# Hex-Lee/gluon-e2e-asr

Hardware: NVIDIA B200
Metric: ctc_fwd_bwd_valid_frames_per_sec (higher is better)
Workload: dtype f64

## Files before the change

gluon_e2e_asr_b200/csrc/ctcb.cu:

```cuda
#include <cuda_runtime.h>
#include <dlfcn.h>
#include <stdarg.h>
#include <stdio.h>
#include <stdlib.h>
#include <string.h>

#include <mutex>
#include <new>
#include <utility>
#include <vector>

#include "ctcb.h"
#include "ctcb_dlpack.h"
#include "ctcb_kernels.cuh"
#include "ctcb_meet.cuh"
#include "ctcb_grad2.cuh"
#include "ctcb_proj.cuh"

struct ctcb_mailbox {
    int device = 0, rank = 0, world = 0;
    double* local = nullptr;
    void* opened[ctcb::kMailMaxRanks] = {};
    ctcb::MailboxDev dev{};
    ctcb::MailboxDev* dev_d = nullptr;
// ... 14 lines not shown
    cudaLaunchAttribute attr[1];
    attr[0].id = cudaLaunchAttributeProgrammaticStreamSerialization;
    attr[0].val.programmaticStreamSerializationAllowed = 1;
    cfg.attrs = attr; cfg.numAttrs = programmatic ? 1 : 0;
    const ctcb::MailboxDev* md = g_xchg.mb->dev_d;
    cudaLaunchKernelEx(&cfg, ctcb::k_mailbox_exchange, md, g_xchg.values, g_xchg.count, g_xchg.out, 0);
    g_xchg = PendingXchg{};
    return true;
}
thread_local const ctcb_proj_t* g_proj = nullptr;
struct DecodeRequest { int32_t* tokens; int32_t* lengths; int unk; };
thread_local const DecodeRequest* g_decode = nullptr;
thread_local bool g_recompute = false;
thread_local cudaEvent_t* g_prof_events = nullptr;
thread_local int g_prof_count = 0;

enum Opt { OPT_WALK_P, OPT_WALK_NW, OPT_WALK_STAGES, OPT_OVERLAP, OPT_FUSED, OPT_WALK_PER_SM, OPT_EMIT_STAGED,
           OPT_GRAD_STAGED, OPT_MEET, OPT_GRAD2, OPT_GRAD2_BLOCKS, OPT_WALK_HW_WAIT, OPT_GRAD2_OCC, OPT_PROJ_CTAS, OPT_PROJ_DBG, OPT_PROJ_OVERLAP, OPT_MEET_FWD, OPT_WALK_PDL, OPT_GRAD_POLL_NS, OPT_COUNT };
const char* const kOptNames[OPT_COUNT] = {"walk_p", "walk_nw", "walk_stages", "overlap", "fused", "walk_per_sm",
                                          "emit_staged", "grad_staged", "meet", "grad2", "grad2_blocks", "walk_hw_wait", "grad2_occ", "proj_ctas", "proj_dbg", "proj_overlap", "meet_fwd", "walk_pdl", "grad_poll_ns"};
struct Options {
    int v[OPT_COUNT];
    Options() {
        for (int i = 0; i < OPT_COUNT; ++i) {
            char name[64] = "CTCB_";
            size_t k = 5;
            for (const char* c = kOptNames[i]; *c && k + 1 < sizeof(name); ++c) name[k++] = (char)(*c >= 'a' && *c <= 'z' ? *c - 32 : *c);
            name[k] = 0;
            const char* e = getenv(name);
            v[i] = e ? atoi(e) : -1;
// ... 226 lines not shown
}

bool is_device_ptr(const void* ptr) {
    if (!ptr) return true;
    cudaPointerAttributes at{};
    if (cudaPointerGetAttributes(&at, ptr) != cudaSuccess) { cudaGetLastError(); return false; }
    return at.type == cudaMemoryTypeDevice || at.type == cudaMemoryTypeManaged;
}
void* pinned_device_alias(const void* ptr) {
    if (!ptr) return nullptr;
    cudaPointerAttributes at{};
    if (cudaPointerGetAttributes(&at, ptr) != cudaSuccess) { cudaGetLastError(); return nullptr; }
    return at.type == cudaMemoryTypeHost ? at.devicePointer : nullptr;
}

}

extern "C" {

int ctcb_version(void) { return CTCB_VERSION; }
const char* ctcb_last_error(void) { return g_err; }
int ctcb_last_launch_count(void) { return g_launches; }
int ctcb_last_walk_config(int32_t* p, int32_t* nw) {
    if (p) *p = g_walk_p;
    if (nw) *nw = g_walk_nw;
    return CTCB_OK;
}

int ctcb_last_grad_kernel(void) { return g_grad_kernel; }

int ctcb_set_option(const char* name, int32_t value) {
    if (!name) return fail(CTCB_INVALID_VALUE, "option name is NULL");
    for (int i = 0; i < OPT_COUNT; ++i)
// ... 183 lines not shown
        if (lay.off_hA + need <= lay.total) {
            if (p->status) CUDA_TRY(cudaMemsetAsync(p->status, 0, sizeof(int32_t) * (size_t)p->B, stream));
            ctcb::MeetArgs ma{dp, w.hA, lay.NB};
            using MeetFn = void (*)(ctcb::MeetArgs);
            const MeetFn mfn = mp == 1 ? ctcb::k_meet<1> : mp == 2 ? ctcb::k_meet<2> : ctcb::k_meet<4>;
            const size_t msm = ctcb::meet_smem_layout(mp, p->V, lay.Lp).total;
            CUDA_TRY(ensure_dynamic_smem(reinterpret_cast<const void*>(mfn), msm));
            g_walk_p = mp; g_walk_nw = 1; g_grad_kernel = 3;
            mfn<<<p->B, 256, msm, stream>>>(ma);
            mark(stream);
            if (launch_pending_xchg(stream)) mark(stream);
            CUDA_TRY(cudaGetLastError());
            return CTCB_OK;
        }
    }
    if (phases & PH_FORWARD) {
        if (p->status) CUDA_TRY(cudaMemsetAsync(p->status, 0, sizeof(int32_t) * (size_t)p->B, stream));
        const WalkEntry* we = lay.walk;
        if (!we) return fail(CTCB_UNSUPPORTED, "no walker configuration for Lmax=%d", p->Lmax);
        g_walk_p = we->P; g_walk_nw = we->NW;
        int stages = 0;
        if (!pick_stages(lay.W, we->NW, lay.fused ? lay.Lp : 0, &stages))
            return fail(CTCB_UNSUPPORTED, "Lmax=%d V=%d: the emission ring does not fit in shared memory", p->Lmax, p->V);
        const WalkFn wfn = (bf && lay.fused) ? we->fused_bf16[need_grad ? 1 : 0] : we->fn[lay.fused][need_grad ? 1 : 0];
        size_t smem = ctcb::walk_smem_bytes(lay.W, we->NW, stages, lay.fused ? lay.Lp : 0);
        if (lay.fused && need_grad && (phases & PH_BACKWARD) && overlap_allowed(p->B, true)) {
            int dev = 0, nsm = 148;
            cudaGetDevice(&dev);
            cudaDeviceGetAttribute(&nsm, cudaDevAttrMultiProcessorCount, dev);
            int per_sm = (2 * p->B + nsm - 1) / nsm;
// ... 36 lines not shown
                }
#undef EMIT_NQ
#undef EMIT_LAUNCH
            }
            mark(stream);
            return CTCB_OK;
        };
        const bool xchg = !(phases & PH_BACKWARD) && launch_pending_xchg(stream);
        if (xchg) mark(stream);
        const bool beside = g_proj && !need_grad && !xchg && !g_prof_events && opt(OPT_PROJ_OVERLAP) != 0;
        const bool meet_fwd = !need_grad && (opt(OPT_MEET_FWD) >= 0 ? opt(OPT_MEET_FWD) != 0 : (p->B <= 148 && !beside));
        if (meet_fwd) CUDA_TRY(cudaMemsetAsync(w.meetcnt, 0, sizeof(int) * (size_t)p->B, stream));
        auto launch_walk = [&](bool after_xchg, bool beside_proj) -> int {
            ctcb::WalkArgs wa{dp, w, p->T, stages, p->blank, p->loss, p->loss_sum, nullptr, 0, 1, 0, 0, 0};
            wa.beside_proj = beside_proj ? 1 : 0;
            const bool pdl = lay.fused && !after_xchg && !beside_proj && opt(OPT_WALK_PDL) != 0;
            wa.pdl_wait = pdl ? 1 : 0;
            wa.meet = meet_fwd ? 1 : 0;
            wa.hw_wait = opt(OPT_WALK_HW_WAIT) >= 0 ? opt(OPT_WALK_HW_WAIT) : (2 * p->B > 148 ? 1 : 0);
            wa.publish = ((phases & PH_BACKWARD) && !g_prof_events && overlap_allowed(p->B, lay.fused != 0)) ? 1 : 2;
            const int wthreads = (we->NW + (lay.fused ? ctcb::kFusedProducers + 1 : 1)) * 32;
            cudaLaunchConfig_t cfg{};
            cfg.gridDim = dim3(p->B, (need_grad || meet_fwd) ? 2 : 1); cfg.blockDim = dim3(wthreads); cfg.dynamicSmemBytes = smem; cfg.stream = stream;
            cudaLaunchAttribute attr[1];
            attr[0].id = cudaLaunchAttributeProgrammaticStreamSerialization;
            attr[0].val.programmaticStreamSerializationAllowed = 1;
            cfg.attrs = attr; cfg.numAttrs = (after_xchg || pdl) ? 1 : 0;
            CUDA_TRY(cudaLaunchKernelEx(&cfg, wfn, wa));
            mark(stream);
            return CTCB_OK;
// ... 4 lines not shown
        if (int rc = launch_walk((xchg && lay.fused != 0) || beside, beside)) return rc;
        if (g_recompute) {
            CUDA_TRY(ctcb::launch_proj_occ(dp, w, stream));
            mark(stream);
        }
        if (g_decode) {
            const size_t dsm = 2 * sizeof(int) * (size_t)p->T;
            if (dsm > 48 * 1024) CUDA_TRY(ensure_dynamic_smem(reinterpret_cast<const void*>(ctcb::k_greedy_collapse), dsm));
            ctcb::k_greedy_collapse<<<p->B, 256, dsm, stream>>>(w.tflag, w.ntile, p->data_lengths, p->data_lengths_dtype, p->T, p->blank,
                                                                g_decode->unk, g_decode->tokens, g_decode->lengths);
            mark(stream);
        }
    }
    if (phases & PH_BACKWARD) {
        ctcb::GradArgs ga{dp, w};
        const int gpairs = p->Lmax + 1;
        const int gch = gpairs <= 32 ? 1 : gpairs <= 64 ? 2 : gpairs <= 128 ? 4 : gpairs <= 256 ? 8 : gpairs <= 512 ? 16 : 0;
        size_t gsm = ctcb::grad_smem_bytes(lay.Lp, 32 * gch);
        int gthreads = 128;
        if (gsm > 200 * 1024) return fail(CTCB_UNSUPPORTED, "Lmax=%d too long for the gradient kernel", p->Lmax);
        int vec = pick_vec(p->logits, p->logits_stride_t, p->logits_row_offsets ? 0 : p->logits_stride_b, p->V, esz);
        const int gvec = pick_vec(p->grad, p->grad_stride_t, p->grad_stride_b, p->V, esz);
        if (gvec < vec) vec = gvec;
        const int ch = gch;
        const int units = (p->V / vec + 31) / 32;
        const int xq = units <= 1 ? 1 : units <= 2 ? 2 : units <= 4 ? 4 : 0;
        const dim3 ggrid(p->B, lay.NB);
        using GradFn = void (*)(ctcb::GradArgs);
        GradFn gfn = nullptr;
#define GRAD_X(V_, C_, T_) (xq == 1 ? ctcb::k_grad<V_, C_, 1, 0, T_> : xq == 2 ? ctcb::k_grad<V_, C_, 2, 0, T_> : \
// ... 876 lines not shown
```

gluon_e2e_asr_b200/csrc/ctcb_kernels.cuh:

```cuda
#pragma once
#include <cuda_bf16.h>
#include <cuda_runtime.h>
#include <stdint.h>

namespace ctcb {

constexpr int kG = 8;
constexpr int kEC = 10;
constexpr int kD = 100;
constexpr int kDrift = 200;
constexpr int kZeroE = -(1 << 28);
constexpr float kLog2e = 1.4426950408889634f;
constexpr double kLn2 = 0.6931471805599453094;
constexpr float kMinLog2 = -100.0f;
constexpr int kMaxStages = 16;

enum : int { UTT_INFEASIBLE = 1, UTT_BAD_LABEL = 2, UTT_LEN_CLAMPED = 4, UTT_WIDE_LOGITS = 8 };
constexpr long long kSpinLimit = 4000000000LL;
enum : int { DT_I32 = 0, DT_I64 = 1, DT_F32 = 2, DT_F64 = 3 };

struct Problem {
    int T, B, V, Lmax, blank, label_pad;
    const float* logits; long long st_t, st_b;
    const long long* row_off;
// ... 496 lines not shown
    long long* trace;
    int hw_wait;
    int publish;
    int meet;
    int pdl_wait;
    int beside_proj;
};

#ifdef CTCB_TRACE
#define CTCB_TP(id) do { if (a.trace && blockIdx.x == 0 && lane == 0) \
    a.trace[((size_t)(blockIdx.y * 32 + warp) * 4096 + (size_t)n * 8 + (id))] = clock64(); } while (0)
#else
#define CTCB_TP(id) do { } while (0)
#endif

struct HaloMeta { double lm; int el; int R; int F; int pad; };
constexpr int kHaloDepth = 16;

constexpr int kFusedProducers = 2;

__host__ __device__ inline size_t walk_smem_bytes(int W, int NW, int stages, int fused_Lp = 0) {
    return (size_t)stages * kEC * W * sizeof(double) + 2 * kMaxStages * sizeof(uint64_t) +
           (size_t)NW * kHaloDepth * kG * sizeof(double) + (size_t)NW * kHaloDepth * sizeof(HaloMeta) +
           (size_t)NW * sizeof(int) + 64 + (fused_Lp ? 16 + kFusedProducers * 64 + (size_t)fused_Lp * sizeof(int) : 0);
}

template <int P, int NW, int DIR, bool HIST, bool FUSED, typename LT = float>
__device__ __forceinline__ void walk_dir(const WalkArgs& a, unsigned char* smem_raw, int Tb, int Lb, int uflags) {
    constexpr int PW = 32 * P;
    constexpr unsigned FULL = 0xffffffffu;
    const Workspace& w = a.w;
    const int b = blockIdx.x;
    const int tid = threadIdx.x, lane = tid & 31, warp = tid >> 5;
    const int W = w.W, NS = a.stages;
    const int NQ = (Tb + kG - 1) / kG;
    const int rlast = Tb - (NQ - 1) * kG;
    const bool meet = !HIST && a.meet && NQ >= 2;
    const int Mblk = (NQ + 1) / 2;
    const int NQr = meet ? (DIR ? NQ - Mblk : Mblk) : NQ;
    if (!HIST && DIR == 1 && !meet) return;
    const uint32_t stage_bytes = (uint32_t)W * kEC * 8u;

    const uint32_t ring = smem_u32(smem_raw);
// ... 4 lines not shown
    const uint32_t prog = meta + NW * kHaloDepth * (uint32_t)sizeof(HaloMeta);
    const uint32_t lsum = (prog + NW * 4 + 7u) & ~7u;
    int* slab = reinterpret_cast<int*>(smem_raw + (lsum - ring) + 32 + kFusedProducers * 64);

    if (tid == 0) {
        for (int s = 0; s < NS; ++s) { mbar_init(&full[s], 1); mbar_init(&empty[s], NW); }
        asm volatile("fence.mbarrier_init.release.cluster;" ::: "memory");
        sts_s32(lsum + 8, 0);
        if (FUSED) for (int q = 0; q < kFusedProducers * 8; ++q) sts_f64(lsum + 16 + q * 8, 0.0);
    }
    if (tid < NW) sts_s32(prog + tid * 4, 0);
    __syncthreads();

    if (FUSED && warp >= NW && warp < NW + kFusedProducers) {
        const Problem& p = a.p;
        constexpr int CPL = 16;
        const int q = warp - NW, V = p.V;
        const int fj = lane >> 2, qk = lane & 3;
        const int cpl = (V + 3) >> 2, col0 = qk * cpl;
        const LT* base = utt_logits<LT>(p, b);
        const float kMinProb = 7.888609052210118e-31f;
        auto load_blk = [&](int n, float (&x)[CPL]) {
            const int t = (DIR ? NQ - 1 - n : n) * kG + fj;
            const LT* row = base + (long long)t * p.st_t + col0;
            const bool valid = t < Tb;
#pragma unroll
            for (int i = 0; i < CPL; ++i) x[i] = (valid && i < cpl && col0 + i < V) ? ldx(row + i) : -INFINITY;
        };
        float cur[CPL], nxt[CPL];
        double ls = 0.0;
        bool floored = false;
        int n = q;
        if (n < NQr) load_blk(n, cur);
#pragma unroll 1
        for (; n < NQr; n += kFusedProducers) {
            if (n + kFusedProducers < NQr) load_blk(n + kFusedProducers, nxt);
            const int t = (DIR ? NQ - 1 - n : n) * kG + fj;
            const bool valid = t < Tb;
            float mx = cur[0];
#pragma unroll
            for (int i = 1; i < CPL; ++i) mx = fmaxf(mx, cur[i]);
            mx = fmaxf(mx, __shfl_xor_sync(FULL, mx, 1));
            mx = fmaxf(mx, __shfl_xor_sync(FULL, mx, 2));
            float e[CPL], sm = 0.0f;
#pragma unroll
            for (int i = 0; i < CPL; ++i) {
                e[i] = valid ? fast_ex2((cur[i] - mx) * kLog2e) : 0.0f;
                sm += e[i];
// ... 43 lines not shown
            if (c1 > 0) dl[__popc(m0) + __popc(m1 & below)] = make_int2(lane + 32, r1);
            w.runv[(size_t)b * 64 + lane] = make_int2(r0, r0 + c0);
            w.runv[(size_t)b * 64 + lane + 32] = make_int2(r1, r1 + c1);
            for (int j = 0; j < Lb; ++j) {
                const int v = slab[j];
                if (v == lane) rank[j] = r0++;
                else if (v == lane + 32) rank[j] = r1++;
            }
            if (lane == 0) {
                dl[nd] = make_int2(-1, Lb);
                w.nd[b] = nd; w.Tb[b] = Tb; w.Lb[b] = Lb; w.flags[b] = uflags;
            }
            __syncwarp();
            if (lane == 0) st_release_gpu(w.gprog + 4 * b + 2, w.stamp);
        }
        if (HIST && lane == 0 && a.publish) {
            int* gp = w.gprog + 4 * b + DIR;
            const uint32_t last_prog = prog + (NW - 1) * 4;
            int seen = 0;
            while (seen < NQ) {
                const int v = lds_acquire(last_prog);
                if (v > seen) { st_release_gpu(gp, v); seen = v; }
                else __nanosleep(a.publish == 2 ? 4000 : 128);
            }
        }
        (void)p;
        return;
    }

    if (!FUSED && warp == NW) {
        const double* Eb = w.E + (size_t)b * w.NB * W * kEC;
        int tile_seen = -1;
        auto issue = [&](int n, int st) {
            const int blk = DIR ? NQ - 1 - n : n;
            if (a.beside_proj && (blk >> 4) != tile_seen) {
                const int* f = w.tflag + (size_t)b * w.ntile + (blk >> 4);
                const long long t0 = clock64();
                while (ld_acquire_gpu(f) == 0 && clock64() - t0 < kSpinLimit) __nanosleep(256);
// ... 75 lines not shown
    const uint32_t nb_meta = meta + (warp > 0 ? warp - 1 : 0) * kHaloDepth * (uint32_t)sizeof(HaloMeta);
    const uint32_t nb_prog = prog + (warp > 0 ? warp - 1 : 0) * 4;
    double pm = 0.0;
    int c_el = 0, c_R = 0, c_F = 0;
    int Rout = 0, Fout = 0;

    int st = 0, ph = 0;
    uint32_t stage_base = ring;
#pragma unroll 1
    for (int n = 0; n < NQr; ++n) {
        const int blk = DIR ? NQ - 1 - n : n;
        const int ns = blk == NQ - 1 ? rlast : kG;
        const uint32_t par = (uint32_t)(n & (kHaloDepth - 1));
        CTCB_TP(0);
        mbar_wait(&full[st], ph);
        const int j0 = DIR ? ns - 1 : 0;
        double yb, yl[P];
        yb = lds_f64(stage_base + bcol + (uint32_t)j0 * 8u);
#pragma unroll
        for (int p = 0; p < P; ++p) yl[p] = lds_f64(stage_base + ccol[p] + (uint32_t)j0 * 8u);
        int bad = 0;
        {
            constexpr unsigned LO = (1023u - kDrift) << 20, SPAN = (2u * kDrift + 1u) << 20;
#pragma unroll
            for (int p = 0; p < P; ++p) {
                const unsigned hb = (unsigned)__double2hiint(bm[p]), hl = (unsigned)__double2hiint(lm[p]);
                bad |= (int)(hb != 0u) & (int)(hb - LO >= SPAN);
                bad |= (int)(hl != 0u) & (int)(hl - LO >= SPAN);
            }
        }
// ... 150 lines not shown
                step(j, nj, DIR ? 0u - (uint32_t)j * 8u : (uint32_t)j * 8u);
            }
        } else {
#pragma unroll 1
            for (int jj = 0; jj < ns; ++jj) {
                const int j = DIR ? ns - 1 - jj : jj;
                const int nj = jj + 1 < ns ? (DIR ? j - 1 : j + 1) : -1;
                step(j, nj, DIR ? 0u - (uint32_t)j * 8u : (uint32_t)j * 8u);
            }
        }
        CTCB_TP(4);
        __syncwarp();
        if (lane == 31) {
            if (NW > 1 || (FUSED && HIST)) sts_release(prog + warp * 4, n + 1);
            mbar_arrive(&empty[st]);
        }
        CTCB_TP(5);
        CTCB_TP(6);
        stage_base += stage_bytes;
        if (++st == NS) { st = 0; ph ^= 1; stage_base = ring; }
        if (HIST) { hch += DIR ? -kHistStep : kHistStep; och += DIR ? -kOffStep : kOffStep; }
    }

    if (meet) {
        MeetSlot* mine = w.meet + ((size_t)b * 2 + DIR) * (NW * PW) + g0;
#pragma unroll
        for (int p = 0; p < P; ++p) {
            double vb = bm[p], vl = lm[p];
            if (DIR) {
                const double prev = p == 0 ? pm : lm[p - 1];
                const double t0 = fma(bm[p], flb[p], lm[p]);
                vb = fma(prev, fb[p], bm[p]);
                vl = fma(prev, fls[p], t0);
            }
            MeetSlot ms;
            ms.ob = vb != 0.0 ? eb[p] + dexp(vb) : kZeroE; ms.vb = vb != 0.0 ? dmant(vb) : 0.0;
            ms.ol = vl != 0.0 ? el[p] + dexp(vl) : kZeroE; ms.vl = vl != 0.0 ? dmant(vl) : 0.0;
            mine[p] = ms;
// ... 64 lines not shown
                    lz = lds_f64(lsum);
                }
                const double nll = -kLn2 * ((double)eb[p] + log2(sb) - lz);
                a.loss[b] = (float)nll;
                if (a.loss_sum) atomicAdd(a.loss_sum, nll);
            }
        }
    }
}

template <int P, int NW, bool HIST, bool FUSED, typename LT = float>
__global__ void __launch_bounds__((NW + (FUSED ? kFusedProducers + 1 : 1)) * 32) k_walk(WalkArgs a) {
    extern __shared__ __align__(128) unsigned char smem_raw[];
    if (a.pdl_wait) asm volatile("griddepcontrol.wait;" ::: "memory");
    const int b = blockIdx.x;
    if (!FUSED) {
        asm volatile("griddepcontrol.launch_dependents;" ::: "memory");
        if (a.beside_proj) {
            if (threadIdx.x == 0) {
                const long long t0 = clock64();
                while (ld_acquire_gpu(a.w.gprog + 4 * b + 2) != a.w.stamp && clock64() - t0 < kSpinLimit) __nanosleep(256);
            }
            __syncthreads();
        }
        const int flags = __ldcg(a.w.flags + b), Tb = __ldcg(a.w.Tb + b), Lb = __ldcg(a.w.Lb + b);
        if (flags & UTT_INFEASIBLE) return;
        if (blockIdx.y == 0) walk_dir<P, NW, 0, HIST, false>(a, smem_raw, Tb, Lb, flags);
        else                 walk_dir<P, NW, 1, HIST, false>(a, smem_raw, Tb, Lb, flags);
        return;
    }
    const Problem& p = a.p;
    const Workspace& w = a.w;
    const int tid = threadIdx.x, nthr = blockDim.x;
    __shared__ int s_L, s_rep, s_flags;
    if (tid == 0) {
        w.gprog[4 * b + blockIdx.y] = 0;
        if (blockIdx.y == 0) { w.gprog[4 * b + 2] = 0; w.gprog[4 * b + 3] = 0; }
        __threadfence();
        s_L = p.Lmax; s_rep = 0; s_flags = 0;
    }
    __syncthreads();
    asm volatile("griddepcontrol.launch_dependents;" ::: "memory");
    int Tb = p.T, lenflags = 0;
    if (p.data_len) {
        long long t64 = load_as_int(p.data_len, p.data_len_dtype, b);
        if (t64 < 0) { t64 = 0; lenflags = UTT_LEN_CLAMPED; }
        if (t64 > p.T) { t64 = p.T; lenflags = UTT_LEN_CLAMPED; }
        Tb = (int)t64;
    }
    int L;
    if (p.label_len) {
        long long l64 = load_as_int(p.label_len, p.label_len_dtype, b);
        if (l64 < 0) { l64 = 0; lenflags = UTT_LEN_CLAMPED; }
        if (l64 > p.Lmax) { l64 = p.Lmax; lenflags = UTT_LEN_CLAMPED; }
        L = (int)l64;
    } else {
        for (int j = tid; j < p.Lmax; j += nthr)
            if (load_as_int(p.labels, p.label_dtype, b * p.lst_b + j * p.lst_l) == p.label_pad) atomicMin(&s_L, j);
        __syncthreads();
        L = s_L;
    }
    int* slab;
    {
        const size_t stage_bytes = (size_t)w.W * kEC * 8;
        size_t off = (size_t)a.stages * stage_bytes + 2 * kMaxStages * sizeof(uint64_t) +
                     (size_t)NW * kHaloDepth * kG * 8 + (size_t)NW * kHaloDepth * sizeof(HaloMeta) + (size_t)NW * 4;
        off = (off + 7) & ~(size_t)7;
        slab = reinterpret_cast<int*>(smem_raw + off + 32 + kFusedProducers * 64);
    }
    {
        int bad = 0;
        for (int j = tid; j < L; j += nthr) {
            long long v = load_as_int(p.labels, p.label_dtype, b * p.lst_b + j * p.lst_l);
            if (v < 0 || v >= p.V || v == p.blank) bad = 1;
            slab[j] = (int)(v < 0 ? 0 : (v >= p.V ? p.V - 1 : v));
        }
        if (bad) atomicOr(&s_flags, UTT_BAD_LABEL);
    }
    __syncthreads();
    {
        int rep = 0;
        for (int j = tid + 1; j < L; j += nthr) rep += slab[j] == slab[j - 1];
        if (rep) atomicAdd(&s_rep, rep);
    }
    __syncthreads();
    int flags = s_flags | lenflags;
    if (Tb <= 0 || L + s_rep > Tb) flags |= UTT_INFEASIBLE;
    if (blockIdx.y == 0 && tid == 0) {
        if (p.status) p.status[b] = flags;
        if (flags & UTT_INFEASIBLE) {
            p.loss[b] = 0.0f;
            w.Tb[b] = Tb; w.Lb[b] = L; w.flags[b] = flags; w.nd[b] = 0;
            st_release_gpu(w.gprog + 4 * b + 2, w.stamp);
        } else if (!HIST) {
            w.Tb[b] = Tb; w.Lb[b] = L; w.flags[b] = flags;
        }
    }
    if (flags & UTT_INFEASIBLE) return;
    if (blockIdx.y == 0) walk_dir<P, NW, 0, HIST, true, LT>(a, smem_raw, Tb, L, flags);
    else                 walk_dir<P, NW, 1, HIST, true, LT>(a, smem_raw, Tb, L, flags);
}

constexpr int kMailMaxRanks = 16, kMailMaxCount = 6, kMailRow = 8;
constexpr int kMailMaxLag = 8;
struct MailboxDev {
    double* peer[kMailMaxRanks];
    unsigned long long* counter;
    int rank, world;
    int lag;
};

__device__ __forceinline__ void mailbox_exchange_warp(const MailboxDev* md, double* values, int count, double* out, int flush, int lane) {
    const MailboxDev& m = *md;
    const unsigned long long k = *m.counter;
    __shared__ double rows[kMailMaxRanks][kMailMaxCount];
// ... 38 lines not shown
    __syncwarp();
    if (lane == 0) {
        for (int c = 0; c < count; ++c) values[c] = 0.0;
        *m.counter = k + 1;
    }
}

#ifndef CTCB_NO_PLAIN_KERNELS
__global__ void __launch_bounds__(32) k_mailbox_exchange(const MailboxDev* m, double* values, int count, double* out, int flush) {
    asm volatile("griddepcontrol.launch_dependents;" ::: "memory");
    mailbox_exchange_warp(m, values, count, out, flush, threadIdx.x);
    if (threadIdx.x == 0) asm volatile("griddepcontrol.wait;" ::: "memory");
}
#endif

struct GradArgs { Problem p; Workspace w; };

template <int VEC, typename LT>
__device__ __forceinline__ void zero_row(LT* row, int V, int lane) {
    using V_t = typename LV<LT, VEC>::type;
    const int nvec = V / VEC;
    V_t z; memset(&z, 0, sizeof(z));
    V_t* rv = reinterpret_cast<V_t*>(row);
    for (int k = lane; k < nvec; k += 32) rv[k] = z;
    for (int v = nvec * VEC + lane; v < V; v += 32) stx(row + v, 0.0f);
}

constexpr int kNoState = INT_MIN / 2;

__device__ __forceinline__ float hw_mant(int h) { return __int_as_float(((h & 0x000fffff) << 3) | 0x3f800000); }
__device__ __forceinline__ void hw_weight(int ha, int hb, int off, float& wgt, int& e) {
    wgt = hw_mant(ha) * hw_mant(hb);
    e = min((unsigned)ha, (unsigned)hb) == 0u ? kNoState : (ha >> 20) + (hb >> 20) + off;
}

constexpr int kGradFramesPerWarp = 2;

__host__ __device__ inline int grad_row_floats(int Lp, int pairs_cap) { return ((Lp > pairs_cap ? Lp : pairs_cap) + 3) & ~3; }
__host__ __device__ inline size_t grad_staged_bytes(int staged_V) { return staged_V ? (size_t)kG * staged_V * 4 + 64 : 0; }
__host__ __device__ inline size_t grad_smem_bytes(int Lp, int pairs_cap, int staged_V = 0) {
    return grad_staged_bytes(staged_V) + (size_t)(Lp + 1) * 8 + (size_t)4 * kGradFramesPerWarp * grad_row_floats(Lp, pairs_cap) * 4 + 16;
}

template <int VEC, int CH, int XQ, int OCC = 0, typename LT = float>
__global__ void __launch_bounds__(XQ < 0 ? 256 : 128, XQ < 0 ? (CH == 16 ? 2 : 3) : ((CH == 0 || CH == 8) ? 5 : (CH <= 4 ? (OCC ? 8 : 1) : 3))) k_grad(GradArgs a) {
    using V_t = typename LV<LT, VEC>::type;
    constexpr int NCH = CH > 0 ? CH : 1, NXQ = XQ > 0 ? XQ : 1;
    constexpr int FPW = XQ < 0 ? 1 : kGradFramesPerWarp, NT = XQ < 0 ? 256 : 128;
    constexpr int F = (CH > 0 && CH <= 4) ? FPW : 1;
    const Problem& p = a.p; const Workspace& w = a.w;
    const int b = blockIdx.x, tid = threadIdx.x, lane = tid & 31, warp = tid >> 5;
    asm volatile("griddepcontrol.launch_dependents;" ::: "memory");
    __shared__ int s_ok;
    constexpr bool STAGED = XQ < 0;
    int Tb_e = 0, Lb_e = 0, fl_e = 0, nd_e = 0, rk_e[NCH];
    extern __shared__ __align__(128) unsigned char gsm_all[];
    if (STAGED) {
        const int st = __ldcg(w.gprog + 4 * b + 2);
        Tb_e = __ldcg(w.Tb + b); Lb_e = __ldcg(w.Lb + b); fl_e = __ldcg(w.flags + b); nd_e = __ldcg(w.nd + b);
        const int* rank_e = w.rank + (size_t)b * w.Lp;
// ... 46 lines not shown
                            utt_logits<LT>(p, b) + (long long)t * p.st_t, (uint32_t)p.V * (uint32_t)sizeof(LT), rbar + j);
            }
        }
    }
    float* gbuf0 = reinterpret_cast<float*>(gsm_raw) + (size_t)warp * FPW * GW;
    int2* s_dl = reinterpret_cast<int2*>(reinterpret_cast<float*>(gsm_raw) + (size_t)4 * kGradFramesPerWarp * GW);
    const int* rank = w.rank + (size_t)b * w.Lp;
    int nd = 0;
    if (cta_live) {
        if (STAGED) nd = nd_e;
        else {
            nd = __ldcg(w.nd + b);
            const int2* dl = w.dl + (size_t)b * (w.Lp + 1);
            for (int j = tid; j <= nd; j += NT) s_dl[j] = __ldcg(dl + j);
        }
        const int* gp = w.gprog + 4 * b;
        if (tid == 0) {
            const long long t0 = clock64();
            const unsigned pns = w.poll_ns > 0 ? (unsigned)w.poll_ns : (STAGED ? 1024u : 256u);
            while (ld_acquire_gpu(gp) < blk + 1 && clock64() - t0 < kSpinLimit) __nanosleep(pns);
            while (ld_acquire_gpu(gp + 1) < NQ - blk && clock64() - t0 < kSpinLimit) __nanosleep(pns);
            if (clock64() - t0 >= kSpinLimit) s_ok = 0;
        }
    }
    __syncthreads();
    if (!s_ok) {
        if (STAGED && lane == 0) {
#pragma unroll
            for (int f = 0; f < FPW; ++f) if (t_first + warp * FPW + f < Tb) mbar_wait(rbar + warp * FPW + f, 0);
        }
        for (int j = warp; j < kG; j += NT / 32) {
            const int t = t_first + j;
            if (t < p.T) {
                LT* grow = grad_row<LT>(p, b, t);
                for (int v = lane; v < p.V; v += 32) stx(grow + v, __int_as_float(0x7fc00000));
            }
        }
        return;
    }

    const int pairs = 32 * w.P * w.NW;
    const size_t blkoff = (size_t)b * w.NB + blk;
    const int2* hA0 = w.hA + blkoff * kG * pairs;
    const int2* hB0 = w.hB + blkoff * kG * pairs;
    const int2* oA = w.oA + blkoff * pairs;
    const int2* oB = w.oB + blkoff * pairs;
    int ibb[NCH], ibl[NCH], ofb[NCH], ofl[NCH], rk[NCH];
    int2 pha[NCH]; int phbb[NCH], phbl[NCH];
    if (STAGED && CH > 0 && cta_live) {
        const int tq = t_first + warp;
#pragma unroll
        for (int c = 0; c < NCH; ++c) {
            const int g = c * 32 + lane;
            ibb[c] = max(Lb - g, 0); ibl[c] = max(Lb - 1 - g, 0);
            pha[c] = make_int2(0, 0); phbb[c] = 0; phbl[c] = 0;
        }
        if (tq < Tb) {
            const int2* A = hA0 + (size_t)(tq - t_first) * pairs + lane;
            const int2* Bh = hB0 + (size_t)(tq - t_first) * pairs;
#pragma unroll
            for (int c = 0; c < NCH; ++c) {
                pha[c] = __ldcg(A + c * 32);
// ... 5 lines not shown
        for (int g = tid; g < 32 * NCH; g += NT) {
            s_off[g] = g < pairs ? __ldcg(oA + g) : make_int2(0, 0);
            s_off[32 * NCH + g] = g < pairs ? __ldcg(oB + g) : make_int2(0, 0);
        }
        __syncthreads();
#pragma unroll
        for (int c = 0; c < NCH; ++c) {
            const int g = c * 32 + lane;
            const int2 oa = s_off[g];
            const int ob = s_off[32 * NCH + ibb[c]].x, ol = s_off[32 * NCH + ibl[c]].y;
            ofb[c] = g <= Lb ? oa.x + ob : kNoState;
            ofl[c] = g < Lb ? oa.y + ol : kNoState;
            rk[c] = g < Lb ? rk_e[c] : g;
        }
        __syncthreads();
    } else if (CH > 0 && cta_live) {
#pragma unroll
        for (int c = 0; c < NCH; ++c) {
            const int g = c * 32 + lane;
            ibb[c] = max(Lb - g, 0); ibl[c] = max(Lb - 1 - g, 0);
            const int2 oa = __ldcg(oA + g);
            const int ob = __ldcg(&oB[ibb[c]].x), ol = __ldcg(&oB[ibl[c]].y);
            ofb[c] = g <= Lb ? oa.x + ob : kNoState;
            ofl[c] = g < Lb ? oa.y + ol : kNoState;
            rk[c] = g < Lb ? (STAGED ? rk_e[c] : __ldcg(rank + g)) : g;
        }
    }
    const int nvec = p.V / VEC;

#pragma unroll
    for (int r = 0; r < FPW / F; ++r) {
        int tt[F]; bool live[F];
        int2 ha[F][NCH]; int hbb[F][NCH], hbl[F][NCH];
        V_t xr[F][NXQ]; float2 fr[F];
#pragma unroll
        for (int f = 0; f < F; ++f) {
            tt[f] = t_first + warp * FPW + r * F + f;
            live[f] = cta_live && tt[f] < Tb;
            fr[f] = make_float2(0.0f, 0.0f);
            if (live[f]) {
                fr[f] = __ldcg(w.fr + (size_t)b * p.T + tt[f]);
                const LT* xrow = utt_logits<LT>(p, b) + (long long)tt[f] * p.st_t;
                if (XQ > 0) {
                    const V_t* xv = reinterpret_cast<const V_t*>(xrow);
#pragma unroll
                    for (int q = 0; q < NXQ; ++q) { const int k = q * 32 + lane; xr[f][q] = k < nvec ? __ldg(xv + k) : LV<LT, VEC>::fill(0.0f); }
                }
                if (CH > 0) {
                    const int2* A = hA0 + (size_t)(tt[f] - t_first) * pairs + lane;
                    const int2* Bh = hB0 + (size_t)(tt[f] - t_first) * pairs;
#pragma unroll
// ... 164 lines not shown
                }
                __syncwarp();
            }
            for (int d = lane; d < nd; d += 32) {
                const int2 e = s_dl[d];
                const int end = s_dl[d + 1].y;
                float occ = 0.0f;
                for (int k = e.y; k < end; ++k) occ += gbuf[k];
                if (e.x == p.blank) occ += zb;
                const float y = fast_ex2(fmaf(ldx(xrow + e.x) - fmx, kLog2e, -flz));
                stx(grow + e.x, head * (y - occ * rZ));
            }
        }
    }
    if (STAGED && lane == 0) tma_store_wait_read();
    if (blockIdx.x == 0 && blockIdx.y == 0 && tid == 0) asm volatile("griddepcontrol.wait;" ::: "memory");
}

#ifndef CTCB_NO_PLAIN_KERNELS
__global__ void __launch_bounds__(256) k_scale_rows(float* grad, long long gst_t, long long gst_b, int T, int B, int V,
                                                    const float* head) {
    const int rows_per_cta = 8, lane = threadIdx.x & 31, warp = threadIdx.x >> 5;
    const long long r = (long long)blockIdx.x * rows_per_cta + warp;
    if (r >= (long long)T * B) return;
    const int b = (int)(r / T), t = (int)(r % T);
    const float h = head[b];
    float* row = grad + b * gst_b + t * gst_t;
    for (int v = lane; v < V; v += 32) row[v] *= h;
}
#endif
// ... 137 lines not shown
```

Baseline: 271.4 million.

## Prefetch logits and history earlier in fused walker and split grad waits

The fused walker now reads the label data and the first block of logits for each producer warp before its setup synchronisation, and replaces shared-memory atomics with warp reductions when computing label length, bad-label and repeat counts. Publication of walker progress switches to a release max-reduction, followed by a final store at the end. The grad kernel waits for only one direction's progress first, issues that direction's history loads, then waits for the other direction. It also raises the min-blocks bound for some configurations. Optional globaltimer tracing hooks are added behind a compile flag. The risks are higher register pressure and subtle ordering problems in the progress protocol.

```diff
diff --git a/gluon_e2e_asr_b200/csrc/ctcb.cu b/gluon_e2e_asr_b200/csrc/ctcb.cu
--- a/gluon_e2e_asr_b200/csrc/ctcb.cu
+++ b/gluon_e2e_asr_b200/csrc/ctcb.cu
@@ -52,6 +52,11 @@
 thread_local bool g_recompute = false;
 thread_local cudaEvent_t* g_prof_events = nullptr;
 thread_local int g_prof_count = 0;
+#ifdef CTCB_STEP_TRACE
+long long* g_trace = nullptr;
+long long g_trace_stride = 0;
+int g_trace_steps = 0, g_trace_next = 0;
+#endif
 
 enum Opt { OPT_WALK_P, OPT_WALK_NW, OPT_WALK_STAGES, OPT_OVERLAP, OPT_FUSED, OPT_WALK_PER_SM, OPT_EMIT_STAGED,
            OPT_GRAD_STAGED, OPT_MEET, OPT_GRAD2, OPT_GRAD2_BLOCKS, OPT_WALK_HW_WAIT, OPT_GRAD2_OCC, OPT_PROJ_CTAS, OPT_PROJ_DBG, OPT_PROJ_OVERLAP, OPT_MEET_FWD, OPT_WALK_PDL, OPT_GRAD_POLL_NS, OPT_COUNT };
@@ -308,9 +313,27 @@
     return at.type == cudaMemoryTypeHost ? at.devicePointer : nullptr;
 }
 
+#ifdef CTCB_STEP_TRACE
+__global__ void k_globaltimer_probe(long long* out, int n) {
+    for (int i = 0; i < n; ++i) out[i] = ctcb::gtimer();
+}
+#endif
+
 }
 
 extern "C" {
+
+#ifdef CTCB_STEP_TRACE
+int ctcb_step_trace(void* buf, int32_t steps, int64_t stride) {
+    g_trace = static_cast<long long*>(buf); g_trace_steps = buf ? steps : 0; g_trace_stride = stride; g_trace_next = 0;
+    return CTCB_OK;
+}
+int ctcb_globaltimer_probe(void* out, int32_t n) {
+    k_globaltimer_probe<<<1, 1>>>(static_cast<long long*>(out), n);
+    CUDA_TRY(cudaDeviceSynchronize());
+    return CTCB_OK;
+}
+#endif
 
 int ctcb_version(void) { return CTCB_VERSION; }
 const char* ctcb_last_error(void) { return g_err; }
@@ -524,6 +547,10 @@
             return CTCB_OK;
         }
     }
+#ifdef CTCB_STEP_TRACE
+    long long* trace = nullptr;
+    if (g_trace && phases == (PH_FORWARD | PH_BACKWARD) && g_trace_next < g_trace_steps) trace = g_trace + g_trace_stride * g_trace_next++;
+#endif
     if (phases & PH_FORWARD) {
         if (p->status) CUDA_TRY(cudaMemsetAsync(p->status, 0, sizeof(int32_t) * (size_t)p->B, stream));
         const WalkEntry* we = lay.walk;
@@ -590,6 +617,9 @@
         auto launch_walk = [&](bool after_xchg, bool beside_proj) -> int {
             ctcb::WalkArgs wa{dp, w, p->T, stages, p->blank, p->loss, p->loss_sum, nullptr, 0, 1, 0, 0, 0};
             wa.beside_proj = beside_proj ? 1 : 0;
+#ifdef CTCB_STEP_TRACE
+            wa.trace = trace;
+#endif
             const bool pdl = lay.fused && !after_xchg && !beside_proj && opt(OPT_WALK_PDL) != 0;
             wa.pdl_wait = pdl ? 1 : 0;
             wa.meet = meet_fwd ? 1 : 0;
@@ -624,6 +654,9 @@
     }
     if (phases & PH_BACKWARD) {
         ctcb::GradArgs ga{dp, w};
+#ifdef CTCB_STEP_TRACE
+        ga.trace = trace;
+#endif
         const int gpairs = p->Lmax + 1;
         const int gch = gpairs <= 32 ? 1 : gpairs <= 64 ? 2 : gpairs <= 128 ? 4 : gpairs <= 256 ? 8 : gpairs <= 512 ? 16 : 0;
         size_t gsm = ctcb::grad_smem_bytes(lay.Lp, 32 * gch);
diff --git a/gluon_e2e_asr_b200/csrc/ctcb_kernels.cuh b/gluon_e2e_asr_b200/csrc/ctcb_kernels.cuh
--- a/gluon_e2e_asr_b200/csrc/ctcb_kernels.cuh
+++ b/gluon_e2e_asr_b200/csrc/ctcb_kernels.cuh
@@ -534,6 +534,17 @@
 #define CTCB_TP(id) do { } while (0)
 #endif
 
+#ifdef CTCB_STEP_TRACE
+__device__ __forceinline__ long long gtimer() {
+    unsigned long long t; asm volatile("mov.u64 %0, %%globaltimer;" : "=l"(t) :: "memory"); return (long long)t;
+}
+#define CTCB_STAMP(tr, idx) do { if (tr) (tr)[idx] = gtimer(); } while (0)
+#define CTCB_STAMP_MAX(tr, idx) do { if (tr) atomicMax(reinterpret_cast<unsigned long long*>(tr) + (idx), (unsigned long long)gtimer()); } while (0)
+#else
+#define CTCB_STAMP(tr, idx) do { } while (0)
+#define CTCB_STAMP_MAX(tr, idx) do { } while (0)
+#endif
+
 struct HaloMeta { double lm; int el; int R; int F; int pad; };
 constexpr int kHaloDepth = 16;
 
@@ -545,8 +556,15 @@
            (size_t)NW * sizeof(int) + 64 + (fused_Lp ? 16 + kFusedProducers * 64 + (size_t)fused_Lp * sizeof(int) : 0);
 }
 
+__device__ __forceinline__ void red_release_gpu_max(int* p, int v) {
+    asm volatile("red.release.gpu.global.max.s32 [%0], %1;" ::"l"(p), "r"(v) : "memory");
+}
+
+constexpr int kFusedCPL = 16;
+
 template <int P, int NW, int DIR, bool HIST, bool FUSED, typename LT = float>
-__device__ __forceinline__ void walk_dir(const WalkArgs& a, unsigned char* smem_raw, int Tb, int Lb, int uflags) {
+__device__ __forceinline__ void walk_dir(const WalkArgs& a, unsigned char* smem_raw, int Tb, int Lb, int uflags,
+                                         const float (&pre)[kFusedCPL], bool pre_ok) {
     constexpr int PW = 32 * P;
     constexpr unsigned FULL = 0xffffffffu;
     const Workspace& w = a.w;
@@ -581,7 +599,7 @@
 
     if (FUSED && warp >= NW && warp < NW + kFusedProducers) {
         const Problem& p = a.p;
-        constexpr int CPL = 16;
+        constexpr int CPL = kFusedCPL;
         const int q = warp - NW, V = p.V;
         const int fj = lane >> 2, qk = lane & 3;
         const int cpl = (V + 3) >> 2, col0 = qk * cpl;
@@ -598,7 +616,15 @@
         double ls = 0.0;
         bool floored = false;
         int n = q;
-        if (n < NQr) load_blk(n, cur);
+        if (n < NQr) {
+            if (pre_ok) {
+                const bool valid = (DIR ? NQ - 1 - n : n) * kG + fj < Tb;
+#pragma unroll
+                for (int i = 0; i < CPL; ++i) cur[i] = valid ? pre[i] : -INFINITY;
+            } else {
+                load_blk(n, cur);
+            }
+        }
 #pragma unroll 1
         for (; n < NQr; n += kFusedProducers) {
             if (n + kFusedProducers < NQr) load_blk(n + kFusedProducers, nxt);
@@ -672,14 +698,14 @@
             __syncwarp();
             if (lane == 0) st_release_gpu(w.gprog + 4 * b + 2, w.stamp);
         }
-        if (HIST && lane == 0 && a.publish) {
+        if (HIST && lane == 0 && a.publish == 1) {
             int* gp = w.gprog + 4 * b + DIR;
             const uint32_t last_prog = prog + (NW - 1) * 4;
             int seen = 0;
-            while (seen < NQ) {
+            while (seen < NQ - 1) {
                 const int v = lds_acquire(last_prog);
-                if (v > seen) { st_release_gpu(gp, v); seen = v; }
-                else __nanosleep(a.publish == 2 ? 4000 : 128);
+                if (v > seen) { if (v < NQ) red_release_gpu_max(gp, v); seen = v; }
+                else __nanosleep(128);
             }
         }
         (void)p;
@@ -785,6 +811,7 @@
         const uint32_t par = (uint32_t)(n & (kHaloDepth - 1));
         CTCB_TP(0);
         mbar_wait(&full[st], ph);
+        if (n == 0 && tid == 0) CTCB_STAMP(a.trace, (size_t)b * 8 + DIR * 4 + 1);
         const int j0 = DIR ? ns - 1 : 0;
         double yb, yl[P];
         yb = lds_f64(stage_base + bcol + (uint32_t)j0 * 8u);
@@ -965,6 +992,7 @@
         if (lane == 31) {
             if (NW > 1 || (FUSED && HIST)) sts_release(prog + warp * 4, n + 1);
             mbar_arrive(&empty[st]);
+            if (n + 1 == NQr && warp == NW - 1) CTCB_STAMP(a.trace, (size_t)b * 8 + DIR * 4 + 2);
         }
         CTCB_TP(5);
         CTCB_TP(6);
@@ -973,6 +1001,10 @@
         if (HIST) { hch += DIR ? -kHistStep : kHistStep; och += DIR ? -kOffStep : kOffStep; }
     }
 
+    if (FUSED && HIST && warp == NW - 1 && lane == 31) {
+        st_release_gpu(a.w.gprog + 4 * blockIdx.x + DIR, lds_relaxed(prog + (NW - 1) * 4));
+        CTCB_STAMP(a.trace, (size_t)b * 8 + DIR * 4 + 3);
+    }
     if (meet) {
         MeetSlot* mine = w.meet + ((size_t)b * 2 + DIR) * (NW * PW) + g0;
 #pragma unroll
@@ -1067,6 +1099,7 @@
     extern __shared__ __align__(128) unsigned char smem_raw[];
     if (a.pdl_wait) asm volatile("griddepcontrol.wait;" ::: "memory");
     const int b = blockIdx.x;
+    if (threadIdx.x == 0) CTCB_STAMP(a.trace, (size_t)b * 8 + blockIdx.y * 4);
     if (!FUSED) {
         asm volatile("griddepcontrol.launch_dependents;" ::: "memory");
         if (a.beside_proj) {
@@ -1078,41 +1111,17 @@
         }
         const int flags = __ldcg(a.w.flags + b), Tb = __ldcg(a.w.Tb + b), Lb = __ldcg(a.w.Lb + b);
         if (flags & UTT_INFEASIBLE) return;
-        if (blockIdx.y == 0) walk_dir<P, NW, 0, HIST, false>(a, smem_raw, Tb, Lb, flags);
-        else                 walk_dir<P, NW, 1, HIST, false>(a, smem_raw, Tb, Lb, flags);
+        const float none[kFusedCPL] = {};
+        if (blockIdx.y == 0) walk_dir<P, NW, 0, HIST, false>(a, smem_raw, Tb, Lb, flags, none, false);
+        else                 walk_dir<P, NW, 1, HIST, false>(a, smem_raw, Tb, Lb, flags, none, false);
         return;
     }
     const Problem& p = a.p;
     const Workspace& w = a.w;
-    const int tid = threadIdx.x, nthr = blockDim.x;
-    __shared__ int s_L, s_rep, s_flags;
-    if (tid == 0) {
-        w.gprog[4 * b + blockIdx.y] = 0;
-        if (blockIdx.y == 0) { w.gprog[4 * b + 2] = 0; w.gprog[4 * b + 3] = 0; }
-        __threadfence();
-        s_L = p.Lmax; s_rep = 0; s_flags = 0;
-    }
-    __syncthreads();
-    asm volatile("griddepcontrol.launch_dependents;" ::: "memory");
-    int Tb = p.T, lenflags = 0;
-    if (p.data_len) {
-        long long t64 = load_as_int(p.data_len, p.data_len_dtype, b);
-        if (t64 < 0) { t64 = 0; lenflags = UTT_LEN_CLAMPED; }
-        if (t64 > p.T) { t64 = p.T; lenflags = UTT_LEN_CLAMPED; }
-        Tb = (int)t64;
-    }
-    int L;
-    if (p.label_len) {
-        long long l64 = load_as_int(p.label_len, p.label_len_dtype, b);
-        if (l64 < 0) { l64 = 0; lenflags = UTT_LEN_CLAMPED; }
-        if (l64 > p.Lmax) { l64 = p.Lmax; lenflags = UTT_LEN_CLAMPED; }
-        L = (int)l64;
-    } else {
-        for (int j = tid; j < p.Lmax; j += nthr)
-            if (load_as_int(p.labels, p.label_dtype, b * p.lst_b + j * p.lst_l) == p.label_pad) atomicMin(&s_L, j);
-        __syncthreads();
-        L = s_L;
-    }
+    const int tid = threadIdx.x, nthr = blockDim.x, lane = tid & 31, warp = tid >> 5;
+    constexpr unsigned FULL = 0xffffffffu;
+    constexpr int NWARPS = NW + kFusedProducers + 1;
+    __shared__ int s_pad[NWARPS], s_bad[NWARPS], s_rep[NWARPS];
     int* slab;
     {
         const size_t stage_bytes = (size_t)w.W * kEC * 8;
@@ -1121,24 +1130,72 @@
         off = (off + 7) & ~(size_t)7;
         slab = reinterpret_cast<int*>(smem_raw + off + 32 + kFusedProducers * 64);
     }
-    {
-        int bad = 0;
-        for (int j = tid; j < L; j += nthr) {
-            long long v = load_as_int(p.labels, p.label_dtype, b * p.lst_b + j * p.lst_l);
-            if (v < 0 || v >= p.V || v == p.blank) bad = 1;
-            slab[j] = (int)(v < 0 ? 0 : (v >= p.V ? p.V - 1 : v));
-        }
-        if (bad) atomicOr(&s_flags, UTT_BAD_LABEL);
-    }
+    long long t64 = p.T, l64 = 0;
+    if (p.data_len) t64 = load_as_int(p.data_len, p.data_len_dtype, b);
+    if (p.label_len) l64 = load_as_int(p.label_len, p.label_len_dtype, b);
+    long long v[P];
+#pragma unroll
+    for (int u = 0; u < P; ++u) {
+        const int j = tid + u * nthr;
+        v[u] = j < p.Lmax ? load_as_int(p.labels, p.label_dtype, b * p.lst_b + j * p.lst_l) : 0;
+    }
+    float pre[kFusedCPL];
+    const bool pre_ok = warp >= NW && warp < NW + kFusedProducers && !p.row_off;
+    if (pre_ok) {
+        const int q = warp - NW, fj = lane >> 2, cpl = (p.V + 3) >> 2, col0 = (lane & 3) * cpl;
+        int t = q * kG + fj, tend = p.T;
+        if (blockIdx.y == 1) {
+            tend = (int)(t64 < 0 ? 0 : (t64 > p.T ? p.T : t64));
+            t = ((tend + kG - 1) / kG - 1 - q) * kG + fj;
+        }
+        const bool in = t >= 0 && t < tend;
+        const LT* row = utt_logits<LT>(p, b) + (long long)(in ? t : 0) * p.st_t + col0;
+#pragma unroll
+        for (int i = 0; i < kFusedCPL; ++i) pre[i] = (in && i < cpl && col0 + i < p.V) ? ldx(row + i) : -INFINITY;
+    }
+    if (tid == 0) {
+        w.gprog[4 * b + blockIdx.y] = 0;
+        if (blockIdx.y == 0) { w.gprog[4 * b + 2] = 0; w.gprog[4 * b + 3] = 0; }
+        __threadfence();
+    }
+    int pad = p.Lmax, bad = p.Lmax;
+#pragma unroll
+    for (int u = 0; u < P; ++u) {
+        const int j = tid + u * nthr;
+        if (j < p.Lmax) {
+            if (v[u] == p.label_pad) pad = min(pad, j);
+            if (v[u] < 0 || v[u] >= p.V || v[u] == p.blank) bad = min(bad, j);
+            slab[j] = (int)(v[u] < 0 ? 0 : (v[u] >= p.V ? p.V - 1 : v[u]));
+        }
+    }
+    pad = __reduce_min_sync(FULL, pad); bad = __reduce_min_sync(FULL, bad);
+    if (lane == 0) { s_pad[warp] = pad; s_bad[warp] = bad; }
     __syncthreads();
+    asm volatile("griddepcontrol.launch_dependents;" ::: "memory");
+    int Tb = (int)t64, lenflags = 0;
+    if (t64 < 0) { Tb = 0; lenflags = UTT_LEN_CLAMPED; }
+    if (t64 > p.T) { Tb = p.T; lenflags = UTT_LEN_CLAMPED; }
+    int L = p.Lmax;
+    bad = p.Lmax;
+#pragma unroll
+    for (int i = 0; i < NWARPS; ++i) { L = min(L, s_pad[i]); bad = min(bad, s_bad[i]); }
+    if (p.label_len) {
+        L = (int)l64;
+        if (l64 < 0) { L = 0; lenflags = UTT_LEN_CLAMPED; }
+        if (l64 > p.Lmax) { L = p.Lmax; lenflags = UTT_LEN_CLAMPED; }
+    }
     {
         int rep = 0;
         for (int j = tid + 1; j < L; j += nthr) rep += slab[j] == slab[j - 1];
-        if (rep) atomicAdd(&s_rep, rep);
+        rep = __reduce_add_sync(FULL, rep);
+        if (lane == 0) s_rep[warp] = rep;
     }
     __syncthreads();
-    int flags = s_flags | lenflags;
-    if (Tb <= 0 || L + s_rep > Tb) flags |= UTT_INFEASIBLE;
+    int reps = 0;
+#pragma unroll
+    for (int i = 0; i < NWARPS; ++i) reps += s_rep[i];
+    int flags = (bad < L ? UTT_BAD_LABEL : 0) | lenflags;
+    if (Tb <= 0 || L + reps > Tb) flags |= UTT_INFEASIBLE;
     if (blockIdx.y == 0 && tid == 0) {
         if (p.status) p.status[b] = flags;
         if (flags & UTT_INFEASIBLE) {
@@ -1150,8 +1207,8 @@
         }
     }
     if (flags & UTT_INFEASIBLE) return;
-    if (blockIdx.y == 0) walk_dir<P, NW, 0, HIST, true, LT>(a, smem_raw, Tb, L, flags);
-    else                 walk_dir<P, NW, 1, HIST, true, LT>(a, smem_raw, Tb, L, flags);
+    if (blockIdx.y == 0) walk_dir<P, NW, 0, HIST, true, LT>(a, smem_raw, Tb, L, flags, pre, pre_ok);
+    else                 walk_dir<P, NW, 1, HIST, true, LT>(a, smem_raw, Tb, L, flags, pre, pre_ok);
 }
 
 constexpr int kMailMaxRanks = 16, kMailMaxCount = 6, kMailRow = 8;
@@ -1220,7 +1277,12 @@
 }
 #endif
 
-struct GradArgs { Problem p; Workspace w; };
+struct GradArgs {
+    Problem p; Workspace w;
+#ifdef CTCB_STEP_TRACE
+    long long* trace;
+#endif
+};
 
 template <int VEC, typename LT>
 __device__ __forceinline__ void zero_row(LT* row, int V, int lane) {
@@ -1249,7 +1311,7 @@
 }
 
 template <int VEC, int CH, int XQ, int OCC = 0, typename LT = float>
-__global__ void __launch_bounds__(XQ < 0 ? 256 : 128, XQ < 0 ? (CH == 16 ? 2 : 3) : ((CH == 0 || CH == 8) ? 5 : (CH <= 4 ? (OCC ? 8 : 1) : 3))) k_grad(GradArgs a) {
+__global__ void __launch_bounds__(XQ < 0 ? 256 : 128, XQ < 0 ? (CH == 16 ? 2 : 3) : ((CH == 0 || CH == 8) ? 5 : (CH <= 4 ? (OCC ? 8 : (XQ == 1 || XQ == 2 ? 5 : 1)) : 3))) k_grad(GradArgs a) {
     using V_t = typename LV<LT, VEC>::type;
     constexpr int NCH = CH > 0 ? CH : 1, NXQ = XQ > 0 ? XQ : 1;
     constexpr int FPW = XQ < 0 ? 1 : kGradFramesPerWarp, NT = XQ < 0 ? 256 : 128;
@@ -1326,16 +1388,109 @@
             const int2* dl = w.dl + (size_t)b * (w.Lp + 1);
             for (int j = tid; j <= nd; j += NT) s_dl[j] = __ldcg(dl + j);
         }
-        const int* gp = w.gprog + 4 * b;
+    }
+    int ibb[NCH], ibl[NCH], ofb[NCH], ofl[NCH], rk[NCH];
+    int s_tt[F]; bool s_live[F];
+    int2 s_ha[F][NCH]; int s_hbb[F][NCH], s_hbl[F][NCH];
+    V_t s_xr[F][NXQ]; float2 s_fr[F];
+    constexpr bool SPLIT = !STAGED && CH > 0 && F == FPW && OCC == 0;
+    const bool a_first = 2 * blk + 1 <= NQ;
+    const int* gp = w.gprog + 4 * b;
+    if (SPLIT) {
+#pragma unroll
+        for (int f = 0; f < F; ++f) {
+            s_tt[f] = t_first + warp * FPW + f;
+            s_live[f] = cta_live && s_tt[f] < Tb;
+            s_fr[f] = make_float2(0.0f, 0.0f);
+        }
+    }
+    if (cta_live) {
+        if (SPLIT) {
+#pragma unroll
+            for (int f = 0; f < F; ++f) {
+                if (s_live[f] && XQ > 0) {
+                    const int nvec = p.V / VEC;
+                    const V_t* xv = reinterpret_cast<const V_t*>(utt_logits<LT>(p, b) + (long long)s_tt[f] * p.st_t);
+#pragma unroll
+                    for (int q = 0; q < NXQ; ++q) { const int k = q * 32 + lane; s_xr[f][q] = k < nvec ? __ldg(xv + k) : LV<LT, VEC>::fill(0.0f); }
+                }
+            }
+#pragma unroll
+            for (int c = 0; c < NCH; ++c) {
+                const int g = c * 32 + lane;
+                ibb[c] = max(Lb - g, 0); ibl[c] = max(Lb - 1 - g, 0);
+                rk[c] = g < Lb ? __ldcg(rank + g) : g;
+            }
+        }
         if (tid == 0) {
             const long long t0 = clock64();
             const unsigned pns = w.poll_ns > 0 ? (unsigned)w.poll_ns : (STAGED ? 1024u : 256u);
-            while (ld_acquire_gpu(gp) < blk + 1 && clock64() - t0 < kSpinLimit) __nanosleep(pns);
-            while (ld_acquire_gpu(gp + 1) < NQ - blk && clock64() - t0 < kSpinLimit) __nanosleep(pns);
+            if (SPLIT) {
+                const int* g1 = a_first ? gp : gp + 1;
+                const int need = a_first ? blk + 1 : NQ - blk;
+                while (ld_acquire_gpu(g1) < need && clock64() - t0 < kSpinLimit) __nanosleep(pns);
+            } else {
+                while (ld_acquire_gpu(gp) < blk + 1 && clock64() - t0 < kSpinLimit) __nanosleep(pns);
+                while (ld_acquire_gpu(gp + 1) < NQ - blk && clock64() - t0 < kSpinLimit) __nanosleep(pns);
+                CTCB_STAMP(a.trace, (size_t)8 * p.B + 2 * ((size_t)b * w.NB + blk));
+            }
             if (clock64() - t0 >= kSpinLimit) s_ok = 0;
         }
     }
     __syncthreads();
+    if (SPLIT && cta_live) {
+        const int pairs = 32 * w.P * w.NW;
+        const size_t blkoff = (size_t)b * w.NB + blk;
+        const int2* hA0 = w.hA + blkoff * kG * pairs;
+        const int2* hB0 = w.hB + blkoff * kG * pairs;
+        const int2* oA = w.oA + blkoff * pairs;
+        const int2* oB = w.oB + blkoff * pairs;
+        auto issue = [&](bool alpha, int (&hx)[F][NCH], int (&hy)[F][NCH], int (&ox)[NCH], int (&oy)[NCH]) {
+#pragma unroll
+            for (int f = 0; f < F; ++f) {
+                if (!s_live[f]) continue;
+                const int2* H = (alpha ? hA0 : hB0) + (size_t)(s_tt[f] - t_first) * pairs;
+#pragma unroll
+                for (int c = 0; c < NCH; ++c) {
+                    hx[f][c] = __ldcg(&H[alpha ? c * 32 + lane : ibb[c]].x);
+                    hy[f][c] = __ldcg(&H[alpha ? c * 32 + lane : ibl[c]].y);
+                }
+            }
+            const int2* O = alpha ? oA : oB;
+#pragma unroll
+            for (int c = 0; c < NCH; ++c) { ox[c] = __ldcg(&O[alpha ? c * 32 + lane : ibb[c]].x); oy[c] = __ldcg(&O[alpha ? c * 32 + lane : ibl[c]].y); }
+        };
+        int h1x[F][NCH], h1y[F][NCH], o1x[NCH], o1y[NCH], h2x[F][NCH], h2y[F][NCH], o2x[NCH], o2y[NCH];
+        issue(a_first, h1x, h1y, o1x, o1y);
+        if (tid == 0) {
+            const long long t0 = clock64();
+            const unsigned pns = w.poll_ns > 0 ? (unsigned)w.poll_ns : (STAGED ? 1024u : 256u);
+            if (s_ok) {
+                const int* g2 = a_first ? gp + 1 : gp;
+                const int need = a_first ? NQ - blk : blk + 1;
+                while (ld_acquire_gpu(g2) < need && clock64() - t0 < kSpinLimit) __nanosleep(pns);
+                if (clock64() - t0 >= kSpinLimit) s_ok = 0;
+            }
+            CTCB_STAMP(a.trace, (size_t)8 * p.B + 2 * blkoff);
+        }
+        __syncthreads();
+        issue(!a_first, h2x, h2y, o2x, o2y);
+#pragma unroll
+        for (int f = 0; f < F; ++f)
+            if (s_live[f]) s_fr[f] = __ldcg(w.fr + (size_t)b * p.T + s_tt[f]);
+#pragma unroll
+        for (int c = 0; c < NCH; ++c) {
+#pragma unroll
+            for (int f = 0; f < F; ++f) {
+                s_ha[f][c] = a_first ? make_int2(h1x[f][c], h1y[f][c]) : make_int2(h2x[f][c], h2y[f][c]);
+                s_hbb[f][c] = a_first ? h2x[f][c] : h1x[f][c];
+                s_hbl[f][c] = a_first ? h2y[f][c] : h1y[f][c];
+            }
+            const int g = c * 32 + lane;
+            ofb[c] = g <= Lb ? (a_first ? o1x[c] + o2x[c] : o2x[c] + o1x[c]) : kNoState;
+            ofl[c] = g < Lb ? (a_first ? o1y[c] + o2y[c] : o2y[c] + o1y[c]) : kNoState;
+        }
+    }
     if (!s_ok) {
         if (STAGED && lane == 0) {
 #pragma unroll
@@ -1357,7 +1512,6 @@
     const int2* hB0 = w.hB + blkoff * kG * pairs;
     const int2* oA = w.oA + blkoff * pairs;
     const int2* oB = w.oB + blkoff * pairs;
-    int ibb[NCH], ibl[NCH], ofb[NCH], ofl[NCH], rk[NCH];
     int2 pha[NCH]; int phbb[NCH], phbl[NCH];
     if (STAGED && CH > 0 && cta_live) {
         const int tq = t_first + warp;
@@ -1393,7 +1547,7 @@
             rk[c] = g < Lb ? rk_e[c] : g;
         }
         __syncthreads();
-    } else if (CH > 0 && cta_live) {
+    } else if (!SPLIT && CH > 0 && cta_live) {
 #pragma unroll
         for (int c = 0; c < NCH; ++c) {
             const int g = c * 32 + lane;
@@ -1412,8 +1566,18 @@
         int tt[F]; bool live[F];
         int2 ha[F][NCH]; int hbb[F][NCH], hbl[F][NCH];
         V_t xr[F][NXQ]; float2 fr[F];
-#pragma unroll
-        for (int f = 0; f < F; ++f) {
+        if (SPLIT) {
+#pragma unroll
+            for (int f = 0; f < F; ++f) {
+                tt[f] = s_tt[f]; live[f] = s_live[f]; fr[f] = s_fr[f];
+#pragma unroll
+                for (int q = 0; q < NXQ; ++q) xr[f][q] = s_xr[f][q];
+#pragma unroll
+                for (int c = 0; c < NCH; ++c) { ha[f][c] = s_ha[f][c]; hbb[f][c] = s_hbb[f][c]; hbl[f][c] = s_hbl[f][c]; }
+            }
+        }
+#pragma unroll
+        for (int f = 0; f < F && !SPLIT; ++f) {
             tt[f] = t_first + warp * FPW + r * F + f;
             live[f] = cta_live && tt[f] < Tb;
             fr[f] = make_float2(0.0f, 0.0f);
@@ -1608,6 +1772,7 @@
         }
     }
     if (STAGED && lane == 0) tma_store_wait_read();
+    if (cta_live && lane == 0) CTCB_STAMP_MAX(a.trace, (size_t)8 * p.B + 2 * ((size_t)b * w.NB + blk) + 1);
     if (blockIdx.x == 0 && blockIdx.y == 0 && tid == 0) asm volatile("griddepcontrol.wait;" ::: "memory");
 }
 
```

New measurement: 279.2 million (median of 6 runs). 1.03x the previous value.
